# wushan270/mit-6.824-2015

Hardware: AMD Instinct MI355X
Metric: word-count input GB/s (whole node) and % of HBM roofline at 1/2/4/8 MI355X (higher is better)
Workload: dtype u8

## Files before the change

mit-6.824-2015_amd/csrc/wcg_agg.h:

```cpp
#pragma once
#include "wcg_common.h"
#include "wcg_lds_table.h"
#include "wcg_map.h"

namespace wcg {

constexpr int AGG_NT = 1024;
constexpr u32 AGG_BATCH = AGG_NT * 4;
constexpr int AGG_W = 2;
constexpr int AGG_NB = 3350;
constexpr u32 AGG_SLACK_UNITS = AGG_BATCH + 8;
constexpr u32 AGG_MAX_SRC = 256;
constexpr u32 AGG_Q = 128;
constexpr u32 AGG_OVF_CAP = 4096;
constexpr int AGG_SPILL = 0, AGG_EMIT = 1;
#ifndef WCG_AGG_PROBES
#define WCG_AGG_PROBES 2
#endif
constexpr int AGG_PROBES = WCG_AGG_PROBES;
#ifndef WCG_AGG_SPEC_K1
#define WCG_AGG_SPEC_K1 0
#endif
constexpr bool AGG_SPEC_K1 = WCG_AGG_SPEC_K1;
#ifndef WCG_AGG_SPEC_MED
// ... 3 lines not shown
#define WCG_AGG_KINDS 1
#endif
#ifndef WCG_AGG_ABLATE
#define WCG_AGG_ABLATE 0
#endif

struct AggArgs {
    const u64* pool;
    const u32* region_len;
    u64 region_cap;
    u32 P;
    u32 nsrc;
    u32 slices;
    u32 pm;
    u32 slices_m;
    u32 nbi;
    u32 ls_nreg;
    u32 rstride, rmod;
    u32 P1;
    int mode;
    GEntry* gtab;
    u64 gmask;
    DevState* st;
    const u64* map_stats;
    u64* spill;
    u64 spill_cap;
    u32* spill_len;
    Rec* emit;
    u64 emit_cap;
    Rec* ovf;
    u32 ovf_cap;
    u64* clk;
    uint16_t* flist;
};

#ifndef WCG_AGG2_LDSHASH
#define WCG_AGG2_LDSHASH 0
#endif
__device__ __forceinline__ u32 agg_hash(u64 k0, u64 k1) {
    if (WCG_AGG2_LDSHASH) return lds_hash(k0, k1) * 0x9E3779B1u;
    return (u32)(key_hash(k0, k1) >> 32);
}

__device__ __forceinline__ void agg_decode(const u64 (&u)[6], u64 (&k0)[4], u64 (&k1)[4], u64 (&c)[4], bool (&v)[4],
                                           u32 (&nu)[4]) {
#pragma unroll
    for (int k = 0; k < 4; k++) {
        const u32 T = (u32)(u[k] >> 56);
        const bool head = T >= 0x41;
        v[k] = T != 0 && (head || (T & 0x1F) < 8);
        const u64 last = head ? u[k + 1] : u[k];
        k0[k] = head ? u[k] : (u[k] & ~U_CNT);
        k1[k] = head ? (u[k + 1] & ~U_CNT) : 0;
        const bool hc = (last & U_CNT) != 0;
        c[k] = hc ? (head ? u[k + 2] : u[k + 1]) : 1;
        nu[k] = (head ? 2u : 1u) + (hc ? 1u : 0u);
    }
}

__device__ __forceinline__ void agg_decode_short(const u64 (&u)[6], u64 (&k0)[4], u64 (&k1)[4], u64 (&c)[4], bool (&v)[4],
                                                 u32 (&nu)[4]) {
#pragma unroll
    for (int k = 0; k < 4; k++) {
        v[k] = (u[k] >> 56) != 0;
        const bool hc = (u[k] & U_CNT) != 0;
        k0[k] = u[k] & ~U_CNT;
// ... 10 lines not shown
        const bool hc = (u[k + 1] & U_CNT) != 0;
        k0[k] = u[k];
        k1[k] = u[k + 1] & ~U_CNT;
        c[k] = hc ? u[k + 2] : 1;
        nu[k] = hc ? 3u : 2u;
    }
}

#define WCG_AGG_SET_OPS(S)                                                                      \
    __device__ __forceinline__ void agg_load_##S(const v4u* q, v4u& x0, v4u& x1, v4u& x2) {     \
        asm volatile("global_load_dwordx4 %0, %3, off ; wcg-load " #S "0\n\t"                   \
                     "global_load_dwordx4 %1, %3, off offset:16 ; wcg-load " #S "1\n\t"         \
                     "global_load_dwordx4 %2, %3, off offset:32 ; wcg-load " #S "2"              \
                     : "=&v"(x0), "=&v"(x1), "=&v"(x2) : "v"(q) : "memory");                    \
    }                                                                                           \
    template <int N>                                                                            \
    __device__ __forceinline__ void agg_wait_##S(v4u& x0, v4u& x1, v4u& x2) {                   \
        asm volatile("s_waitcnt vmcnt(%3) ; wcg-wait " #S " %0 %1 %2"                            \
                     : "+v"(x0), "+v"(x1), "+v"(x2) : "n"(N) : "memory");                       \
    }
WCG_AGG_SET_OPS(A)
WCG_AGG_SET_OPS(B)
WCG_AGG_SET_OPS(C)
#undef WCG_AGG_SET_OPS
#ifndef WCG_AGG_SETS1
#define WCG_AGG_SETS1 2
#endif
#ifndef WCG_AGG_SETS2
#define WCG_AGG_SETS2 2
#endif

template <int MODE, int KIND>
__device__ __forceinline__ u64 agg_one(const AggArgs& a, u32 bi, u64 (*tk0)[AGG_W], u64 (*tk1)[AGG_W], u64 (*tcnt)[AGG_W], u32* rlen_s,
                       u32* bstart, u32& spos, u64 (*wsum)[4]) {
    const int tid = threadIdx.x;
    LdsTable<AGG_NB, u64, AGG_W> tab{tk0, tk1, tcnt};
    constexpr bool emit = MODE == AGG_EMIT;
    u32 p, s, sl;
    if (bi < a.pm * a.slices) { p = bi % a.pm; s = bi / a.pm; sl = a.slices; }
    else { const u32 b2 = bi - a.pm * a.slices, nm = a.P - a.pm; p = a.pm + b2 % nm; s = b2 / nm; sl = a.slices_m; }
#ifdef WCG_AGG_MREV
    if (p >= a.pm && a.pm < a.P) p = a.P - 1 - (p - a.pm);
#endif
    u32 k0_, k1_, wbase, wstep;
    if (!emit) {
        k0_ = (u32)(((u64)a.nsrc * s) / sl); k1_ = (u32)(((u64)a.nsrc * (s + 1)) / sl);
        wbase = 0; wstep = 1;
    } else {
        k0_ = 0; k1_ = a.nsrc;
        wbase = p / AGG_Q; wstep = a.P1;
    }
    const u32 nk = k1_ - k0_;
    auto region = [&](u32 k) -> u64 { return (u64)(wbase + k * wstep) * a.rstride + p % a.rmod; };
    constexpr u32 WB = 256;
    for (u32 k = tid; k < nk; k += AGG_NT) rlen_s[k] = a.region_len[region(k0_ + k)];
    __syncthreads();
    if (tid == 0) {
        u32 t = 0;
        for (u32 k = 0; k < nk; k++) { bstart[k] = t; t += (rlen_s[k] + WB - 1) / WB; }
        bstart[nk] = t;
        spos = 0;
    }
    __syncthreads();
    const u32 nbat = bstart[nk];
    if (nbat == 0) {
        if (!emit && tid == 0 && a.spill_len) a.spill_len[bi] = 0;
        return 0;
    }
    tab.init(tid, AGG_NT);
    __syncthreads();
    u64 my_global = 0;
    u64* const sp = emit ? nullptr : a.spill + (u64)bi * a.spill_cap;
    auto overflow = [&](u64 k0, u64 k1, u64 c, u32 nu) {
        if (emit) {
            const u32 pos = atomicAdd(&spos, 1u);
            if (pos < a.ovf_cap) { a.ovf[(u64)blockIdx.x * a.ovf_cap + pos] = inline_rec(k0, k1, c); return; }
        } else {
            const u32 pos = atomicAdd(&spos, nu);
            if (pos + nu <= a.spill_cap) {
                u64 e[3];
                const u64 f = c > 1 ? U_CNT : 0;
                if (key_short(k0)) { e[0] = k0 | f; e[1] = c; }
                else { e[0] = k0; e[1] = k1 | f; e[2] = c; }
                for (u32 j = 0; j < nu; j++) sp[pos + j] = e[j];
                return;
            }
            for (u64 j = pos; j < a.spill_cap; j++) sp[j] = 0;
        }
        my_global++;
        ginsert(a.gtab, a.gmask, k0, k1, gslot(key_hash(k0, k1)), c, a.st);
    };
    const u32 wave = (u32)__builtin_amdgcn_readfirstlane(tid >> 6), lane = tid & 63;
    constexpr u32 WSTRIDE = AGG_NT / 64;
    const bool per_wave = !emit;
    auto advance = [&](u32& k, u32& b, u32 step) {
        if (per_wave) {
            b += step / WSTRIDE;
            while (k < nk && b >= bstart[k + 1] - bstart[k]) { k += WSTRIDE; b = 0; }
            return;
        }
        b += step;
        while (k < nk) {
            const u32 nbk = bstart[k + 1] - bstart[k];
            if (b < nbk) break;
            b -= nbk;
            k++;
        }
    };
    auto batch_ptr = [&](u32 k, u32 b) -> const v4u* {
        const bool live = k < nk;
        const u64 i = (live ? (u64)b * WB : 0) + 4 * lane;
        return reinterpret_cast<const v4u*>(a.pool + region(k0_ + (live ? k : 0)) * a.region_cap + i);
    };
    auto unit = [](const v4u& x, int h) -> u64 { return h ? ((u64)x.w << 32 | x.z) : ((u64)x.y << 32 | x.x); };
    auto process = [&](u32 k, u32 b, const v4u& x0, const v4u& x1, const v4u& x2) {
        u64 u[6] = {unit(x0, 0), unit(x0, 1), unit(x1, 0), unit(x1, 1), unit(x2, 0), unit(x2, 1)};
        const u32 i0 = b * WB + 4 * lane, len = rlen_s[k];
#pragma unroll
        for (int j = 0; j < 6; j++) u[j] = i0 + j < len ? u[j] : 0;
        if (WCG_AGG_ABLATE == 1) { asm volatile("" ::"v"(u[0] ^ u[1] ^ u[2] ^ u[3] ^ u[4] ^ u[5])); return; }
        u64 k0[4], k1[4], c[4];
        bool v[4];
        u32 nu[4];
        if (KIND == 1) agg_decode_short(u, k0, k1, c, v, nu);
        else if (KIND == 2) agg_decode_medium(u, k0, k1, c, v, nu);
        else agg_decode(u, k0, k1, c, v, nu);
        if (WCG_AGG_ABLATE == 4) {
#pragma unroll
            for (int j = 0; j < 4; j++) v[j] = v[j] && key_short(k0[j]);
        }
        if (WCG_AGG_ABLATE == 2) {
            u32 x = 0;
#pragma unroll
            for (int j = 0; j < 4; j++) x ^= v[j] ? lds_hash(k0[j], k1[j]) + (u32)c[j] : 0u;
            asm volatile("" ::"v"(x));
            return;
        }
        static_assert(4 % AGG_PROBES == 0, "probe groups split a lane's 4 units");
        constexpr bool SPEC = KIND == 2 ? WCG_AGG_SPEC_MED : AGG_SPEC_K1;
#pragma unroll
        for (int j = 0; j < 4; j += AGG_PROBES) {
            typename decltype(tab)::Probe pr[AGG_PROBES];
#pragma unroll
            for (int q = 0; q < AGG_PROBES; q++) {
                const u32 h = emit ? agg_hash(k0[j + q], k1[j + q]) : lds_hash(k0[j + q], k1[j + q]);
                if (!v[j + q]) continue;
                if (SPEC) tab.start_k1(h, KIND == 2 || !key_short(k0[j + q]), pr[q]);
                else tab.start(h, pr[q]);
            }
#pragma unroll
            for (int q = 0; q < AGG_PROBES; q++) {
                if (!v[j + q]) continue;
                const bool ok = SPEC ? tab.template finish_k1<KIND>(k0[j + q], k1[j + q], pr[q], c[j + q])
                                     : tab.template finish<KIND>(k0[j + q], k1[j + q], pr[q], c[j + q]);
                if (!ok) overflow(k0[j + q], k1[j + q], c[j + q], nu[j + q]);
            }
        }
    };
    constexpr int NSETS = emit ? WCG_AGG_SETS2 : WCG_AGG_SETS1;
    static_assert(NSETS == 2 || NSETS == 3, "k_agg's batch walk names two or three register sets");
    u32 kA = 0, bA = 0, kB, bB, kC = 0, bC = 0;
    if (per_wave) { kA = wave; bA = (u32)-1; advance(kA, bA, WSTRIDE); }
    else advance(kA, bA, wave);
    kB = kA; bB = bA;
    advance(kB, bB, WSTRIDE);
    v4u a0, a1, a2, b0, b1, b2, c0, c1, c2;
    agg_load_A(batch_ptr(kA, bA), a0, a1, a2);
    agg_load_B(batch_ptr(kB, bB), b0, b1, b2);
    if (NSETS == 3) {
        kC = kB; bC = bB;
        advance(kC, bC, WSTRIDE);
        agg_load_C(batch_ptr(kC, bC), c0, c1, c2);
        while (kA < nk) {
            agg_wait_A<6>(a0, a1, a2);
            process(kA, bA, a0, a1, a2);
            kA = kC; bA = bC;
            advance(kA, bA, WSTRIDE);
            agg_load_A(batch_ptr(kA, bA), a0, a1, a2);
            if (kB >= nk) break;
            agg_wait_B<6>(b0, b1, b2);
            process(kB, bB, b0, b1, b2);
            kB = kA; bB = bA;
            advance(kB, bB, WSTRIDE);
            agg_load_B(batch_ptr(kB, bB), b0, b1, b2);
            if (kC >= nk) break;
            agg_wait_C<6>(c0, c1, c2);
            process(kC, bC, c0, c1, c2);
            kC = kB; bC = bB;
            advance(kC, bC, WSTRIDE);
            agg_load_C(batch_ptr(kC, bC), c0, c1, c2);
        }
        agg_wait_C<0>(c0, c1, c2);
    } else {
        while (kA < nk) {
            agg_wait_A<3>(a0, a1, a2);
            process(kA, bA, a0, a1, a2);
            kA = kB; bA = bB;
            advance(kA, bA, WSTRIDE);
            agg_load_A(batch_ptr(kA, bA), a0, a1, a2);
            if (kB >= nk) break;
            agg_wait_B<3>(b0, b1, b2);
            process(kB, bB, b0, b1, b2);
            kB = kA; bB = bA;
            advance(kB, bB, WSTRIDE);
            agg_load_B(batch_ptr(kB, bB), b0, b1, b2);
        }
    }
    agg_wait_A<0>(a0, a1, a2);
    agg_wait_B<0>(b0, b1, b2);
    __syncthreads();
    if (!emit && a.flist && !a.spill_cap && WCG_AGG_ABLATE != 3) {
        constexpr u32 NE = AGG_NB * AGG_W;
        uint16_t* const L = a.flist + (u64)bi * NE;
        u32 mine = 0;
        for (int i = tid; i < (int)NE; i += AGG_NT) mine += (&tcnt[0][0])[i] ? 1u : 0u;
        u32 incl = mine;
        for (int d = 1; d < 64; d <<= 1) { const u32 y = __shfl_up(incl, d, 64); if (lane >= (u32)d) incl += y; }
        if (lane == 63) wsum[wave][0] = incl;
        __syncthreads();
        u32 pos = 0, all = 0;
        for (u32 w = 0; w < AGG_NT / 64; w++) { if (w < wave) pos += (u32)wsum[w][0]; all += (u32)wsum[w][0]; }
        pos += incl - mine;
        for (int i = tid; i < (int)NE; i += AGG_NT)
            if ((&tcnt[0][0])[i]) L[pos++] = (uint16_t)i;
        asm volatile("s_waitcnt vmcnt(0)" ::: "memory");
        __syncthreads();
        for (u32 j = tid; j < all; j += AGG_NT) {
            const u32 i = __hip_atomic_load(&L[j], __ATOMIC_RELAXED, __HIP_MEMORY_SCOPE_AGENT);
            const u64 c = (&tcnt[0][0])[i], k0 = (&tk0[0][0])[i], k1 = (&tk1[0][0])[i];
            my_global++;
            ginsert(a.gtab, a.gmask, k0, k1, gslot(key_hash(k0, k1)), c, a.st);
        }
        __syncthreads();
    } else if (!emit) {
        for (int i = tid; i < AGG_NB * AGG_W; i += AGG_NT) {
            const u64 c = (&tcnt[0][0])[i];
            if (!c || WCG_AGG_ABLATE == 3) continue;
            const u64 k0 = (&tk0[0][0])[i], k1 = (&tk1[0][0])[i];
            if (a.spill_cap) { overflow(k0, k1, c, (u32)entry_units(k0, (u32)(c > 1 ? 2 : 1))); continue; }
            my_global++;
            ginsert(a.gtab, a.gmask, k0, k1, gslot(key_hash(k0, k1)), c, a.st);
        }
        __syncthreads();
        if (tid == 0 && a.spill_len) a.spill_len[bi] = spos < a.spill_cap ? spos : (u32)a.spill_cap;
    } else {
        u32 mine = 0;
// ... 23 lines not shown
        for (int i = tid; i < AGG_NB * AGG_W; i += AGG_NT) {
            const u64 c = (&tcnt[0][0])[i];
            if (!c) continue;
            const u64 k0 = (&tk0[0][0])[i], k1 = (&tk1[0][0])[i];
            if (pos < a.emit_cap) a.emit[pos] = inline_rec(k0, k1, c);
            else { my_global++; ginsert(a.gtab, a.gmask, k0, k1, gslot(key_hash(k0, k1)), c, a.st); }
            pos++;
        }
    }
    __syncthreads();
    return my_global;
}

struct AggTabs {
    u64 tk0[AGG_NB][AGG_W];
    u64 tk1[AGG_NB][AGG_W];
    u64 tcnt[AGG_NB][AGG_W];
};
union AggLds {
    AggTabs t;
    LsLds ls;
};
static_assert(LS_NT == AGG_NT, "long_small runs as a k_agg workgroup");
template <int MODE>
__global__ __launch_bounds__(AGG_NT) void k_agg(AggArgs a, MapArgs ma) {
    __shared__ __align__(16) AggLds lds;
    u64 (*const tk0)[AGG_W] = lds.t.tk0;
    u64 (*const tk1)[AGG_W] = lds.t.tk1;
    u64 (*const tcnt)[AGG_W] = lds.t.tcnt;
    __shared__ u32 rlen_s[AGG_MAX_SRC];
    __shared__ u32 bstart[AGG_MAX_SRC + 1];
    __shared__ u32 spos;
    __shared__ u64 wsum[AGG_NT / 64][4];
    const int tid = threadIdx.x;
    const u32 nb = a.nbi;
    if (MODE == AGG_SPILL && a.ls_nreg && blockIdx.x == nb) {
        long_small(ma, a.ls_nreg, lds.ls);
        return;
    }
    const u64 t0 = a.clk ? wall_clock64() : 0;
    if (MODE == AGG_SPILL && blockIdx.x == 0 && tid == 0) { a.st->nrec = 0; a.st->nlong = 0; }
    u64 my_global = 0;
    for (u32 bi = blockIdx.x; bi < nb; bi += gridDim.x)
        if (MODE == AGG_SPILL && WCG_AGG_KINDS && a.pm < a.P)
            my_global += bi < a.pm * a.slices ? agg_one<MODE, 1>(a, bi, tk0, tk1, tcnt, rlen_s, bstart, spos, wsum)
                                              : agg_one<MODE, 2>(a, bi, tk0, tk1, tcnt, rlen_s, bstart, spos, wsum);
        else
            my_global += agg_one<MODE, 0>(a, bi, tk0, tk1, tcnt, rlen_s, bstart, spos, wsum);
    for (int d = 32; d >= 1; d >>= 1) my_global += __shfl_xor(my_global, d, 64);
    u64 ms = 0;
    if (blockIdx.x == 0 && MODE != AGG_EMIT)
        for (u32 w = tid >> 2; w < a.nsrc; w += AGG_NT / 4) ms += a.map_stats[(u64)w * 4 + (tid & 3)];
    for (int d = 32; d >= 4; d >>= 1) ms += __shfl_xor(ms, d, 64);
    if ((tid & 63) < 4) wsum[tid >> 6][tid & 3] = ms + ((tid & 63) == 2 ? my_global : 0);
    __syncthreads();
    if (tid < 4) {
        u64 t = 0;
        for (int w = 0; w < AGG_NT / 64; w++) t += wsum[w][tid];
        u64* dst[4] = {&a.st->tokens, &a.st->lds_hits, &a.st->global_ops, &a.st->long_tokens};
        if (t) atomicAdd(dst[tid], t);
    }
    if (a.clk && tid == 0) { a.clk[2 * blockIdx.x] = t0; a.clk[2 * blockIdx.x + 1] = wall_clock64(); }
}

#ifndef WCG_RP_QB
#define WCG_RP_QB 48
#endif
#ifndef WCG_RP_PREFETCH
#define WCG_RP_PREFETCH 0
#endif
constexpr u32 RP_QB = WCG_RP_QB;
struct RpArgs {
    const u64* pool; const u32* region_len; u64 region_cap;
    u32 P, nsrc, slices;
    const u64* map_stats;
    u64* pool2; u64 cap2; u32* region_len2;
    GEntry* gtab; u64 gmask; DevState* st;
};
#ifndef WCG_RP_MINB
#define WCG_RP_MINB 1
#endif
__global__ __launch_bounds__(AGG_NT, WCG_RP_MINB) void k_rp(RpArgs a) {
    __shared__ u64 sbuf[AGG_Q][RP_QB];
    __shared__ u32 scnt[AGG_Q], sfill[AGG_Q], gpos[AGG_Q], gbase[AGG_Q];
    __shared__ u32 sdirect[AGG_Q];
    __shared__ u64 wsum[AGG_NT / 64][4];
    const u32 b = blockIdx.x, tid = threadIdx.x;
    const u32 p = b % a.P, sl = b / a.P;
    const u32 k0_ = (u32)(((u64)a.nsrc * sl) / a.slices), k1_ = (u32)(((u64)a.nsrc * (sl + 1)) / a.slices);
    u64* const pool2 = a.pool2;
    const u64 cap2 = a.cap2;
    GEntry* const gtab = a.gtab;
    const u64 gmask = a.gmask;
    DevState* const st = a.st;
    if (b == 0) {
// ... 121 lines not shown
```

mit-6.824-2015_amd/csrc/wcg_api.hip:

```cpp
#include <hip/hip_ext.h>
#include <hip/hip_runtime.h>
#include <rccl/rccl.h>

#include <fcntl.h>
#include <sys/stat.h>
#include <unistd.h>

#include <algorithm>
#include <array>
#include <chrono>
#include <cstdio>
#include <cstdlib>
#include <cstring>
#include <memory>
#include <string>
#include <thread>
#include <tuple>
#include <vector>

#include "../../include/wcg.h"
#include "wcg_common.h"
#include "wcg_map.h"
#include "wcg_agg.h"
#include "wcg_reduce.h"
// ... 126 lines not shown
    u64* wg_stats = nullptr; u64 wg_stats_cap = 0;
    u64* llog = nullptr; u64 llog_cap = 0;
    u32* llog_len = nullptr; u64 llog_len_cap = 0;
    u64 chunk = 64ull << 20;
    uint8_t* hb[INGEST_SLOTS] = {};
    uint8_t* db[INGEST_SLOTS] = {};
    uint8_t* dbig = nullptr; u64 dbig_cap = 0;
    hipEvent_t ev_copied[INGEST_SLOTS] = {}, ev_mapped[INGEST_SLOTS] = {};
    std::vector<hipEvent_t> ing_ev;
    double ing[3] = {};
    u64 ing_chunks = 0;
    hipStream_t copy_stream = nullptr;
    std::unique_ptr<TaskPool> readers;
    u64 ingest_bytes = 0;
    bool timing = false;
    bool timing_all = false;
    std::vector<hipEvent_t> ev_pool;
    size_t ev_used = 0;
    std::vector<std::pair<hipEvent_t, hipEvent_t>> map_ev, agg_ev;
    hipEvent_t phase_ev[6] = {};
    u64 map_launches_since_reset = 0;
    int timing_mode = 0;
    std::vector<std::array<hipEvent_t, 5>> phase_jobs;
    bool phase_rec = false;
    std::vector<std::tuple<int, hipEvent_t, hipEvent_t>> xev;
    double acc[10] = {};
    u64 map_launches = 0;
    uint8_t* fr_buf = nullptr;
    FrArgs fr{};
    u32 fr_epoch = 0;
    bool fused_last = false;
    bool pending = false;
    uint16_t* flist = nullptr; u64 flist_cap = 0;
    u64* h_st_dev = nullptr;
    u64* seed = nullptr;
    bool seed_ok = false;
    double seed_rate = -1.0;
    bool job_seeded = false, job_unseeded = false, job_built = false;
    bool last_seeded = false;
    u64 seed_builds = 0;
    u64* d_clk = nullptr;
    u64* d_fclk = nullptr;
    u64* d_stamps = nullptr;
    std::string err;
};

namespace {

#define HIPCHK(ctx, call)                                                                   \
    do {                                                                                    \
        hipError_t e_ = (call);                                                             \
        if (e_ != hipSuccess) {                                                             \
            (ctx)->err = std::string(#call) + ": " + hipGetErrorString(e_);                 \
            return WCG_EHIP;                                                                \
        }                                                                                   \
    } while (0)

#define RC(call)                                                                            \
    do {                                                                                    \
        int rc_ = (call);                                                                   \
        if (rc_) return rc_;                                                                \
    } while (0)

u64 next_pow2(u64 x) {
    u64 p = 1;
    while (p < x) p <<= 1;
// ... 855 lines not shown
    HIPCHK(c, hipMalloc(&c->recA, c->rec_cap * sizeof(Rec)));
    HIPCHK(c, hipMalloc(&c->recB, c->rec_cap * sizeof(Rec)));
    HIPCHK(c, hipHostMalloc(&c->h_cur, EX_MAX_RANKS * sizeof(u64), hipHostMallocDefault));
    HIPCHK(c, hipMalloc(&c->d_per_rank, 2 * EX_MAX_RANKS * sizeof(u64)));
    return wcg_reset(c);
}

int wcg_close(wcg_ctx* c) {
    if (!c) return WCG_EINVAL;
    (void)hipSetDevice(c->device);
    if (c->stream) (void)hipStreamSynchronize(c->stream);
    if (c->copy_stream) (void)hipStreamSynchronize(c->copy_stream);
    if (c->long_stream) (void)hipStreamSynchronize(c->long_stream);
    c->readers.reset();
    if (c->ev_fork) (void)hipEventDestroy(c->ev_fork);
    if (c->ev_join) (void)hipEventDestroy(c->ev_join);
    for (auto e : c->ev_pool) (void)hipEventDestroy(e);
    for (int i = 0; i < INGEST_SLOTS; i++) {
        if (c->ev_copied[i]) (void)hipEventDestroy(c->ev_copied[i]);
    for (auto e : c->ing_ev) (void)hipEventDestroy(e);
        if (c->ev_mapped[i]) (void)hipEventDestroy(c->ev_mapped[i]);
        if (c->hb[i]) (void)hipHostFree(c->hb[i]);
        if (c->db[i]) (void)hipFree(c->db[i]);
    }
    void* bufs[] = {c->gtab, c->ltab, c->arena, c->st, c->recA, c->recB, c->lens, c->d_out,
                    c->d_part, c->owner, c->d_per_rank, c->exp_buf, c->pool, c->region_len, c->wg_stats,
                    c->llog, c->llog_len, c->smp, c->bid, c->spx, c->irec, c->lent, c->lpcur, c->spill, c->spill_len, c->pool2, c->rlen2, c->remit, c->ovf, c->hist, c->spart, c->ikey, c->iidx, c->groups,
                    c->pid, c->d_partb, c->nlpos, c->d_rb, c->d_b0, c->d_jin, c->d_jout, c->jhist, c->dbig,
                    c->ij_in, c->ij_tiles, c->ij_keys, c->ij_units,
                    c->d_xrow, c->xrecv, c->grecv, c->glist, c->llist, c->fr_buf, c->flist,
                    c->top_cand, c->top_rec, c->d_top, c->q_keys, c->q_off, c->q_cnt, c->rs_part, c->d_range,
                    c->bc_key[0], c->bc_key[1], c->bc_idx[0], c->bc_idx[1], c->bc_hist, c->bc_thist, c->bc_rec, c->d_bc,
                    c->bc_q, c->bc_r,
                    c->seed, c->d_clk, c->d_fclk, c->d_stamps};
    for (auto e : c->bc_ev) (void)hipEventDestroy(e);
    if (c->comm) (void)ncclCommDestroy(c->comm);
    for (void* b : bufs) if (b) (void)hipFree(b);
    if (c->h_x) (void)hipHostFree(c->h_x);
    if (c->h_st) (void)hipHostFree(c->h_st);
    if (c->h_cur) (void)hipHostFree(c->h_cur);
    if (c->h_rb) (void)hipHostFree(c->h_rb);
    if (c->copy_stream) (void)hipStreamDestroy(c->copy_stream);
    if (c->own_stream) (void)hipStreamDestroy(c->own_stream);
    if (c->long_stream) (void)hipStreamDestroy(c->long_stream);
    delete c;
    return WCG_OK;
}

int wcg_set_stream(wcg_ctx* c, void* stream) {
    if (!c) return WCG_EINVAL;
    hipStream_t next = stream ? (hipStream_t)stream : c->own_stream;
    if (next != c->stream) {
        int rc = set_dev(c);
        if (rc) return rc;
        hipEvent_t e;
        HIPCHK(c, hipEventCreateWithFlags(&e, hipEventDisableTiming));
        hipError_t r1 = hipEventRecord(e, c->stream);
        hipError_t r2 = r1 == hipSuccess ? hipStreamWaitEvent(next, e, 0) : r1;
        (void)hipEventDestroy(e);
        HIPCHK(c, r2);
        c->stream = next;
    }
    return WCG_OK;
}

int wcg_enable_timing(wcg_ctx* c, int on) {
    if (!c) return WCG_EINVAL;
// ... 63 lines not shown
        }
    }
    const u64* llist = nullptr;
    u64 l16 = c->lslots * sizeof(GEntry) / 16;
    if (c->llist && c->ltab_zero) {
        if (!touched) l16 = 0;
        else {
            RC(read_st());
            if (c->h_st->lnew <= LLIST_CAP) { llist = c->llist; l16 = 2 * c->h_st->lnew; }
        }
    }
    c->map_launches_since_reset = 0;
    if (!clear_g) g16 = 0;
    static_assert(sizeof(GEntry) == 32, "k_clear's listed entries are two 16-byte words");
    static const char* cg_env = getenv("WCG_CLEAR_GRID");
    const u64 cgrid = cg_env ? std::max<u64>(1, (u64)atoi(cg_env)) : grid_for(g16 + l16, 256, c->ncu * 4);
    k_clear<<<(unsigned)cgrid, 256, 0, c->stream>>>(
        reinterpret_cast<uint4*>(c->gtab), g16, reinterpret_cast<uint4*>(c->ltab), l16, c->st, glist, llist);
    HIPCHK(c, hipGetLastError());
    c->gtab_zero = true;
    c->ltab_zero = true;
    c->counts_clean = true;
    c->compacted = c->reduced = c->merged = false;
    c->exp_ready = false;
    c->part_R = 0; c->top_n = 0; c->range_ok = false; c->bc_ok = false; c->bcw_ok = false;
    c->nrec = 0;
    c->out_len = 0;
    c->two_pass_used = false;
    c->imported = false;
    return WCG_OK;
}

int agg_clock_report(wcg_ctx* c, const AggArgs& g, u32 nb1, u64 grid) {
    std::vector<u64> clk(2 * nb1);
    std::vector<u32> rl(grid * g.P);
    HIPCHK(c, hipMemcpyAsync(clk.data(), g.clk, clk.size() * sizeof(u64), hipMemcpyDeviceToHost, c->stream));
    HIPCHK(c, hipMemcpyAsync(rl.data(), g.region_len, rl.size() * sizeof(u32), hipMemcpyDeviceToHost, c->stream));
    HIPCHK(c, hipStreamSynchronize(c->stream));
    u64 t0 = ~0ull, t1 = 0;
    for (u32 b = 0; b < nb1; b++) { t0 = std::min(t0, clk[2 * b]); t1 = std::max(t1, clk[2 * b + 1]); }
    double sd = 0, su = 0, md = 0, mu = 0;
    double kd[2] = {0, 0}, km[2] = {0, 0}, ku[2] = {0, 0};
    u32 kn[2] = {0, 0};
    u32 bmax = 0;
    std::vector<u64> units(nb1, 0);
    for (u32 bi = 0; bi < nb1; bi++) {
        u32 p, s, sl;
        if (bi < g.pm * g.slices) { p = bi % g.pm; s = bi / g.pm; sl = g.slices; }
        else { const u32 b2 = bi - g.pm * g.slices, nm = g.P - g.pm; p = g.pm + b2 % nm; s = b2 / nm; sl = g.slices_m; }
        const u32 k0 = (u32)((grid * s) / sl), k1 = (u32)((grid * (s + 1)) / sl);
        for (u32 k = k0; k < k1; k++) units[bi] += rl[(u64)k * g.P + p];
        const double d = (double)(clk[2 * bi + 1] - clk[2 * bi]);
        sd += d; su += (double)units[bi];
        if (d > md) { md = d; bmax = bi; }
        mu = std::max(mu, (double)units[bi]);
        const int kind = bi >= g.pm * g.slices;
        kd[kind] += d; km[kind] = std::max(km[kind], d); ku[kind] += (double)units[bi]; kn[kind]++;
    }
    static const char* dump = getenv("WCG_AGG_CLOCK_DUMP");
    if (dump) {
        if (FILE* f = fopen(dump, "a")) {
            for (u32 bi = 0; bi < nb1; bi++)
                fprintf(f, "%u %u %llu %.2f %.2f\n", bi, (u32)(bi >= g.pm * g.slices), (unsigned long long)units[bi],
                        (clk[2 * bi] - t0) / 100.0, (clk[2 * bi + 1] - clk[2 * bi]) / 100.0);
            fprintf(f, "--\n");
            fclose(f);
        }
    }
    {
        std::vector<u32> ord(nb1);
        for (u32 i = 0; i < nb1; i++) ord[i] = i;
        std::sort(ord.begin(), ord.end(), [&](u32 x, u32 y) { return clk[2 * x + 1] - clk[2 * x] > clk[2 * y + 1] - clk[2 * y]; });
        for (u32 r = 0; r < std::min<u32>(5, nb1); r++) {
            const u32 bi = ord[r];
            fprintf(stderr, "wcg k_agg clock: slow #%u bi %u (%s) dur %.1f us units %llu\n", r, bi,
                    bi >= g.pm * g.slices ? "medium" : "short", (clk[2 * bi + 1] - clk[2 * bi]) / 100.0,
                    (unsigned long long)units[bi]);
        }
    }
    for (int kind = 0; kind < 2; kind++)
        if (kn[kind])
            fprintf(stderr, "wcg k_agg clock: %s workgroups %u, dur mean %.1f max %.1f us, units mean %.0f\n",
                    kind ? "medium" : "short", kn[kind], kd[kind] / kn[kind] / 100.0, km[kind] / 100.0, ku[kind] / kn[kind]);
    fprintf(stderr, "wcg k_agg clock: span %.1f us, wg dur mean %.1f max %.1f us (bi %u: %llu units, start +%.1f us), "
            "units mean %.0f max %.0f\n", (t1 - t0) / 100.0, sd / nb1 / 100.0, md / 100.0, bmax,
            (unsigned long long)units[bmax], (clk[2 * bmax] - t0) / 100.0, su / nb1, mu);
    return WCG_OK;
}

}

extern "C" {

int wcg_reset(wcg_ctx* c) {
    if (!c) return WCG_EINVAL;
    c->pending = false;
    c->job_seeded = c->job_unseeded = c->job_built = false;
    int rc = set_dev(c);
    if (rc) return rc;
    if (c->timing_mode >= 2 && c->ev_used >= EV_FOLD) {
        HIPCHK(c, hipStreamSynchronize(c->stream));
        sum_events(c, c->acc);
        c->map_ev.clear(); c->agg_ev.clear(); c->phase_jobs.clear(); c->xev.clear();
        c->ev_used = 0;
    }
    RC(reset_tables(c));
    if (c->timing_mode < 2) {
        c->map_ev.clear();
        c->agg_ev.clear();
        c->xev.clear();
        c->ev_used = 0;
// ... 171 lines not shown
    g.P = P; g.nsrc = (u32)grid;
    const u32 min_sl = (u32)((grid + AGG_MAX_SRC - 1) / AGG_MAX_SRC);
    if (split) {
        g.pm = MISS_SHORT_BUCKETS;
        const u32 nm = P - g.pm;
        static const char* ms_env = getenv("WCG_AGG_MSLICES");
        g.slices_m = std::max<u32>(min_sl, std::max<u32>(1, std::min<u32>((u32)grid,
                                   ms_env ? (u32)atoi(ms_env) : (u32)c->ncu / 4 / nm)));
        g.slices = std::max<u32>(min_sl, std::max<u32>(1, std::min<u32>((u32)grid,
                                 (u32)(c->ncu > g.slices_m * nm ? (c->ncu - g.slices_m * nm) / g.pm : 1))));
    } else {
        g.pm = P;
        g.slices_m = 1;
        g.slices = std::max<u32>(1, std::min<u32>((u32)grid, (u32)(c->ncu + P - 1) / P));
        g.slices = std::max<u32>(g.slices, min_sl);
    }
    g.nbi = g.pm * g.slices + (P - g.pm) * g.slices_m;
    g.ls_nreg = small ? (u32)grid : 0u;
    g.rstride = P; g.rmod = P; g.P1 = P; g.mode = AGG_SPILL;
    g.gtab = c->gtab; g.gmask = c->gslots - 1; g.st = c->st;
    g.map_stats = c->wg_stats;
    const u32 nb1 = g.nbi;
    g.spill_cap = 0;
    g.spill = nullptr; g.spill_len = nullptr;
    g.emit = c->remit; g.emit_cap = rec_cap_emit;
    g.ovf = nullptr; g.ovf_cap = 0;
    g.clk = nullptr;
    g.flist = nullptr;
    static const char* fl_env = getenv("WCG_AGG_FLIST");
    if (!two_pass && !(fl_env && atoi(fl_env) == 0)) {
        RC(ensure(c, &c->flist, &c->flist_cap, (u64)nb1 * AGG_NB * AGG_W));
        g.flist = c->flist;
    }
    static const bool agg_clock = getenv("WCG_AGG_CLOCK") != nullptr;
    u64*& d_clk = c->d_clk;
    if (agg_clock && !two_pass) {
        if (!d_clk) HIPCHK(c, hipMalloc(&d_clk, 2 * 65536 * sizeof(u64)));
        g.clk = nb1 <= 65536 ? d_clk : nullptr;
    }
    if (!two_pass) {
        k_agg<AGG_SPILL><<<nb1 + (small ? 1 : 0), AGG_NT, 0, c->stream>>>(g, a);
        HIPCHK(c, hipGetLastError());
        c->counts_clean = true;
        if (g.clk) RC(agg_clock_report(c, g, nb1, grid));
    } else {
    c->two_pass_used = true;
    static const char* rps_env = getenv("WCG_RP_SLICES");
    const u32 sl = std::max<u32>(1, std::min<u32>((u32)grid, rps_env ? (u32)atoi(rps_env) : 2 * g.slices));
    const u32 nrp = P * sl;
    const u64 slice_cap = (u64)cdiv(grid, sl) * a.region_cap;
    u64 cap2 = ((slice_cap * 3 / 2) / AGG_Q + 1024) & ~1ull;
    u64 cap2_env;
    if (cap_env("WCG_RP_CAP2", &cap2_env)) cap2 = std::max<u64>(2, std::min<u64>(cap2_env, 1ull << 31)) & ~1ull;
    RC(ensure(c, &c->pool2, &c->pool2_cap, (u64)nrp * AGG_Q * cap2 + AGG_SLACK_UNITS));
    RC(ensure(c, &c->rlen2, &c->rlen2_cap, (u64)nrp * AGG_Q));
    RpArgs rp;
    rp.pool = c->pool; rp.region_len = c->region_len; rp.region_cap = a.region_cap;
    rp.P = P; rp.nsrc = (u32)grid; rp.slices = sl; rp.map_stats = c->wg_stats;
    rp.pool2 = c->pool2; rp.cap2 = cap2; rp.region_len2 = c->rlen2;
    rp.gtab = c->gtab; rp.gmask = c->gslots - 1; rp.st = c->st;
    k_rp<<<nrp, AGG_NT, 0, c->stream>>>(rp);
    AggArgs g2 = g;
    g2.pool = c->pool2; g2.region_len = c->rlen2; g2.region_cap = cap2;
    g2.P = P * AGG_Q; g2.nsrc = sl; g2.slices = 1;
    g2.pm = g2.P; g2.slices_m = 1; g2.nbi = g2.P;
    g2.rstride = AGG_Q; g2.rmod = AGG_Q; g2.P1 = P; g2.mode = AGG_EMIT;
    const u32 grid2 = std::min<u32>(P * AGG_Q, (u32)c->ncu * 2);
    g2.ovf_cap = AGG_OVF_CAP;
    RC(ensure(c, &c->ovf, &c->ovf_cap, (u64)grid2 * AGG_OVF_CAP));
    g2.ovf = c->ovf;
    g2.ls_nreg = 0;
    k_agg<AGG_EMIT><<<grid2, AGG_NT, 0, c->stream>>>(g2, a);
    HIPCHK(c, hipGetLastError());
    }
// ... 1425 lines not shown
```

Baseline: 1194.

## Add dynamic work-stealing walk to k_agg spill pass with cross-partition helping

Replaces the static slice assignment in the aggregation spill kernel with a per-partition atomic cursor. Workgroups claim chunks of quarter-region items, and workgroups that finish early help the partition with the most remaining work. The long_small path is handed to the first workgroup that wins a ticket instead of getting its own extra block. This targets load imbalance from skewed partitions, at the cost of global atomics, more LDS-table merges when helpers spill the same partition, and a last-block reset of the cursors.

```diff
diff --git a/mit-6.824-2015_amd/csrc/wcg_agg.h b/mit-6.824-2015_amd/csrc/wcg_agg.h
--- a/mit-6.824-2015_amd/csrc/wcg_agg.h
+++ b/mit-6.824-2015_amd/csrc/wcg_agg.h
@@ -59,6 +59,27 @@
     u32 ovf_cap;
     u64* clk;
     uint16_t* flist;
+    u32* cur;
+    u32 help_min;
+};
+
+#ifndef WCG_AGG_PARTS_LOG2
+#define WCG_AGG_PARTS_LOG2 2
+#endif
+constexpr u32 AGG_PARTS_LOG2 = WCG_AGG_PARTS_LOG2, AGG_PARTS = 1u << AGG_PARTS_LOG2;
+static_assert(AGG_PARTS <= 16, "a bucket's items fit 16 bits of lq and 24 of best");
+constexpr u32 AGG_CLAIM = 16;
+constexpr u32 AGG_CLK_WGS = 65536, AGG_CLK_DYN = 2 * AGG_CLK_WGS;
+constexpr u32 AGG_HELP_MIN = 16;
+constexpr u32 AGG_CUR_DONE = MAX_MISS_BUCKETS, AGG_CUR_TICKET = MAX_MISS_BUCKETS + 1, AGG_CUR_WORDS = MAX_MISS_BUCKETS + 2;
+struct AggDyn {
+    u32 lq;
+    u32 lock;
+    u32 dry;
+    u32 nclaim;
+    u32 best;
+    u32 tk;
+    u32 dg[4];
 };
 
 #ifndef WCG_AGG2_LDSHASH
@@ -135,8 +156,9 @@
 
 template <int MODE, int KIND>
 __device__ __forceinline__ u64 agg_one(const AggArgs& a, u32 bi, u64 (*tk0)[AGG_W], u64 (*tk1)[AGG_W], u64 (*tcnt)[AGG_W], u32* rlen_s,
-                       u32* bstart, u32& spos, u64 (*wsum)[4]) {
+                       u32* bstart, u32& spos, u64 (*wsum)[4], AggDyn& dy) {
     const int tid = threadIdx.x;
+    const bool dyn = MODE == AGG_SPILL && a.cur != nullptr;
     LdsTable<AGG_NB, u64, AGG_W> tab{tk0, tk1, tcnt};
     constexpr bool emit = MODE == AGG_EMIT;
     u32 p, s, sl;
@@ -146,7 +168,10 @@
     if (p >= a.pm && a.pm < a.P) p = a.P - 1 - (p - a.pm);
 #endif
     u32 k0_, k1_, wbase, wstep;
-    if (!emit) {
+    if (dyn) {
+        k0_ = 0; k1_ = a.nsrc;
+        wbase = 0; wstep = 1;
+    } else if (!emit) {
         k0_ = (u32)(((u64)a.nsrc * s) / sl); k1_ = (u32)(((u64)a.nsrc * (s + 1)) / sl);
         wbase = 0; wstep = 1;
     } else {
@@ -154,8 +179,24 @@
         wbase = p / AGG_Q; wstep = a.P1;
     }
     const u32 nk = k1_ - k0_;
+    const u32 sh = dyn ? AGG_PARTS_LOG2 : 0u, nki = nk << sh;
     auto region = [&](u32 k) -> u64 { return (u64)(wbase + k * wstep) * a.rstride + p % a.rmod; };
     constexpr u32 WB = 256;
+    if (dyn) {
+        u32 any = 0;
+        for (u32 k = tid; k < nk; k += AGG_NT) { const u32 l = a.region_len[region(k)]; rlen_s[k] = l; any |= l; }
+        any = __syncthreads_or((int)any);
+        if (tid == 0) {
+            const u32 base = atomicAdd(&a.cur[p], any ? AGG_CLAIM : nki);
+            const bool got = any && base < nki;
+            dy.lq = got ? base | (base + AGG_CLAIM < nki ? base + AGG_CLAIM : nki) << 16 : 0u;
+            dy.dry = got ? 0u : 1u;
+            dy.lock = 0; dy.nclaim = 0;
+            spos = 0;
+        }
+        __syncthreads();
+        if (dy.dry) return 0;
+    } else {
     for (u32 k = tid; k < nk; k += AGG_NT) rlen_s[k] = a.region_len[region(k0_ + k)];
     __syncthreads();
     if (tid == 0) {
@@ -165,7 +206,8 @@
         spos = 0;
     }
     __syncthreads();
-    const u32 nbat = bstart[nk];
+    }
+    const u32 nbat = dyn ? 1u : bstart[nk];
     if (nbat == 0) {
         if (!emit && tid == 0 && a.spill_len) a.spill_len[bi] = 0;
         return 0;
@@ -196,10 +238,49 @@
     const u32 wave = (u32)__builtin_amdgcn_readfirstlane(tid >> 6), lane = tid & 63;
     constexpr u32 WSTRIDE = AGG_NT / 64;
     const bool per_wave = !emit;
+    u32 nreg = 0;
+    auto ibeg = [&](u32 k) -> u32 { return (((rlen_s[k >> sh] + WB - 1) / WB) * (k & ((1u << sh) - 1))) >> sh; };
+    auto iend = [&](u32 k) -> u32 { return (((rlen_s[k >> sh] + WB - 1) / WB) * ((k & ((1u << sh) - 1)) + 1)) >> sh; };
+    auto take = [&]() -> u32 {
+        u32 r = nki;
+        if (lane == 0) {
+            u32 q = atomicAdd(&dy.lq, 1u);
+            if ((q & 0xFFFF) < (q >> 16)) r = q & 0xFFFF;
+            else if (!*(volatile u32*)&dy.dry) {
+                if (atomicExch(&dy.lock, 1u) == 0) {
+                    q = atomicAdd(&dy.lq, 1u);
+                    if ((q & 0xFFFF) < (q >> 16)) r = q & 0xFFFF;
+                    else {
+                        const u32 base = atomicAdd(&a.cur[p], AGG_CLAIM);
+                        if (base < nki) {
+                            r = base;
+                            atomicExch(&dy.lq, (base + 1) | (base + AGG_CLAIM < nki ? base + AGG_CLAIM : nki) << 16);
+                        } else *(volatile u32*)&dy.dry = 1;
+                    }
+                    atomicExch(&dy.lock, 0u);
+                } else {
+                    const u32 base = atomicAdd(&a.cur[p], 1u);
+                    if (base < nki) r = base;
+                    else *(volatile u32*)&dy.dry = 1;
+                }
+            }
+        }
+        return (u32)__builtin_amdgcn_readfirstlane(r);
+    };
+    auto take_region = [&]() -> u32 {
+        u32 k;
+        do k = take(); while (k < nki && ibeg(k) == iend(k));
+        if (k < nki) nreg++;
+        return k;
+    };
     auto advance = [&](u32& k, u32& b, u32 step) {
         if (per_wave) {
-            b += step / WSTRIDE;
-            while (k < nk && b >= bstart[k + 1] - bstart[k]) { k += WSTRIDE; b = 0; }
+            if (k >= nki) return;
+            b++;
+            if (b < iend(k)) return;
+            if (dyn) k = take_region();
+            else do k += WSTRIDE; while (k < nk && rlen_s[k] == 0);
+            b = k < nki ? ibeg(k) : 0u;
             return;
         }
         b += step;
@@ -211,14 +292,14 @@
         }
     };
     auto batch_ptr = [&](u32 k, u32 b) -> const v4u* {
-        const bool live = k < nk;
+        const bool live = k < nki;
         const u64 i = (live ? (u64)b * WB : 0) + 4 * lane;
-        return reinterpret_cast<const v4u*>(a.pool + region(k0_ + (live ? k : 0)) * a.region_cap + i);
+        return reinterpret_cast<const v4u*>(a.pool + region(k0_ + (live ? k >> sh : 0)) * a.region_cap + i);
     };
     auto unit = [](const v4u& x, int h) -> u64 { return h ? ((u64)x.w << 32 | x.z) : ((u64)x.y << 32 | x.x); };
     auto process = [&](u32 k, u32 b, const v4u& x0, const v4u& x1, const v4u& x2) {
         u64 u[6] = {unit(x0, 0), unit(x0, 1), unit(x1, 0), unit(x1, 1), unit(x2, 0), unit(x2, 1)};
-        const u32 i0 = b * WB + 4 * lane, len = rlen_s[k];
+        const u32 i0 = b * WB + 4 * lane, len = rlen_s[k >> sh];
 #pragma unroll
         for (int j = 0; j < 6; j++) u[j] = i0 + j < len ? u[j] : 0;
         if (WCG_AGG_ABLATE == 1) { asm volatile("" ::"v"(u[0] ^ u[1] ^ u[2] ^ u[3] ^ u[4] ^ u[5])); return; }
@@ -263,7 +344,8 @@
     constexpr int NSETS = emit ? WCG_AGG_SETS2 : WCG_AGG_SETS1;
     static_assert(NSETS == 2 || NSETS == 3, "k_agg's batch walk names two or three register sets");
     u32 kA = 0, bA = 0, kB, bB, kC = 0, bC = 0;
-    if (per_wave) { kA = wave; bA = (u32)-1; advance(kA, bA, WSTRIDE); }
+    if (dyn) { kA = take_region(); bA = kA < nki ? ibeg(kA) : 0u; }
+    else if (per_wave) { kA = wave; bA = (u32)-1; advance(kA, bA, WSTRIDE); }
     else advance(kA, bA, wave);
     kB = kA; bB = bA;
     advance(kB, bB, WSTRIDE);
@@ -274,19 +356,19 @@
         kC = kB; bC = bB;
         advance(kC, bC, WSTRIDE);
         agg_load_C(batch_ptr(kC, bC), c0, c1, c2);
-        while (kA < nk) {
+        while (kA < nki) {
             agg_wait_A<6>(a0, a1, a2);
             process(kA, bA, a0, a1, a2);
             kA = kC; bA = bC;
             advance(kA, bA, WSTRIDE);
             agg_load_A(batch_ptr(kA, bA), a0, a1, a2);
-            if (kB >= nk) break;
+            if (kB >= nki) break;
             agg_wait_B<6>(b0, b1, b2);
             process(kB, bB, b0, b1, b2);
             kB = kA; bB = bA;
             advance(kB, bB, WSTRIDE);
             agg_load_B(batch_ptr(kB, bB), b0, b1, b2);
-            if (kC >= nk) break;
+            if (kC >= nki) break;
             agg_wait_C<6>(c0, c1, c2);
             process(kC, bC, c0, c1, c2);
             kC = kB; bC = bB;
@@ -295,13 +377,13 @@
         }
         agg_wait_C<0>(c0, c1, c2);
     } else {
-        while (kA < nk) {
+        while (kA < nki) {
             agg_wait_A<3>(a0, a1, a2);
             process(kA, bA, a0, a1, a2);
             kA = kB; bA = bB;
             advance(kA, bA, WSTRIDE);
             agg_load_A(batch_ptr(kA, bA), a0, a1, a2);
-            if (kB >= nk) break;
+            if (kB >= nki) break;
             agg_wait_B<3>(b0, b1, b2);
             process(kB, bB, b0, b1, b2);
             kB = kA; bB = bA;
@@ -311,10 +393,11 @@
     }
     agg_wait_A<0>(a0, a1, a2);
     agg_wait_B<0>(b0, b1, b2);
+    if (dyn && lane == 0 && nreg) atomicAdd(&dy.nclaim, nreg);
     __syncthreads();
     if (!emit && a.flist && !a.spill_cap && WCG_AGG_ABLATE != 3) {
         constexpr u32 NE = AGG_NB * AGG_W;
-        uint16_t* const L = a.flist + (u64)bi * NE;
+        uint16_t* const L = a.flist + (u64)blockIdx.x * NE;
         u32 mine = 0;
         for (int i = tid; i < (int)NE; i += AGG_NT) mine += (&tcnt[0][0])[i] ? 1u : 0u;
         u32 incl = mine;
@@ -404,21 +487,68 @@
     __shared__ u32 bstart[AGG_MAX_SRC + 1];
     __shared__ u32 spos;
     __shared__ u64 wsum[AGG_NT / 64][4];
+    __shared__ AggDyn dy;
     const int tid = threadIdx.x;
     const u32 nb = a.nbi;
-    if (MODE == AGG_SPILL && a.ls_nreg && blockIdx.x == nb) {
-        long_small(ma, a.ls_nreg, lds.ls);
-        return;
-    }
+    const bool dyn = MODE == AGG_SPILL && a.cur != nullptr;
+    bool ls_now = MODE == AGG_SPILL && !dyn && a.ls_nreg && blockIdx.x == nb;
     const u64 t0 = a.clk ? wall_clock64() : 0;
     if (MODE == AGG_SPILL && blockIdx.x == 0 && tid == 0) { a.st->nrec = 0; a.st->nlong = 0; }
     u64 my_global = 0;
-    for (u32 bi = blockIdx.x; bi < nb; bi += gridDim.x)
+    bool first = true;
+    if (dyn && tid == 0) { dy.dg[0] = dy.dg[1] = dy.dg[2] = dy.dg[3] = 0; }
+    for (u32 bi = blockIdx.x; ls_now || bi < nb;) {
+        if (MODE == AGG_SPILL && ls_now) {
+            long_small(ma, a.ls_nreg, lds.ls);
+            if (!dyn) return;
+            ls_now = false;
+            if (tid == 0) dy.dg[3] = 1;
+        } else {
         if (MODE == AGG_SPILL && WCG_AGG_KINDS && a.pm < a.P)
-            my_global += bi < a.pm * a.slices ? agg_one<MODE, 1>(a, bi, tk0, tk1, tcnt, rlen_s, bstart, spos, wsum)
-                                              : agg_one<MODE, 2>(a, bi, tk0, tk1, tcnt, rlen_s, bstart, spos, wsum);
+            my_global += bi < a.pm * a.slices ? agg_one<MODE, 1>(a, bi, tk0, tk1, tcnt, rlen_s, bstart, spos, wsum, dy)
+                                              : agg_one<MODE, 2>(a, bi, tk0, tk1, tcnt, rlen_s, bstart, spos, wsum, dy);
         else
-            my_global += agg_one<MODE, 0>(a, bi, tk0, tk1, tcnt, rlen_s, bstart, spos, wsum);
+            my_global += agg_one<MODE, 0>(a, bi, tk0, tk1, tcnt, rlen_s, bstart, spos, wsum, dy);
+        if (!dyn) { bi += gridDim.x; continue; }
+        if (tid == 0) {
+            const u32 got = dy.nclaim;
+            if (first) dy.dg[0] = got;
+            else { dy.dg[1] += got; dy.dg[2] += got ? 1u : 0u; }
+        }
+        const bool ls_open = first && a.ls_nreg != 0;
+        first = false;
+        if (ls_open) {
+            if (tid == 0)
+                dy.tk = __hip_atomic_load(&a.cur[AGG_CUR_TICKET], __ATOMIC_RELAXED, __HIP_MEMORY_SCOPE_AGENT) ? 1u
+                                                                                                             : atomicAdd(&a.cur[AGG_CUR_TICKET], 1u);
+            __syncthreads();
+            if (dy.tk == 0) { ls_now = true; continue; }
+        }
+        }
+        if (tid == 0) dy.best = 0;
+        __syncthreads();
+        if ((u32)tid < a.P) {
+            const u32 c = __hip_atomic_load(&a.cur[tid], __ATOMIC_RELAXED, __HIP_MEMORY_SCOPE_AGENT);
+            if (c < a.nsrc << AGG_PARTS_LOG2) atomicMax(&dy.best, ((a.nsrc << AGG_PARTS_LOG2) - c) << 8 | (u32)tid);
+        }
+        __syncthreads();
+        const u32 best = dy.best;
+        if ((best >> 8) < a.help_min) break;
+        const u32 hp = best & 255;
+        bi = hp < a.pm ? hp : a.pm * a.slices + (hp - a.pm);
+    }
+    if (dyn) {
+        __syncthreads();
+        if (tid == 0) {
+            __threadfence();
+            dy.tk = atomicAdd(&a.cur[AGG_CUR_DONE], 1u);
+        }
+        __syncthreads();
+        if (dy.tk == gridDim.x - 1) {
+            __threadfence();
+            for (u32 i = tid; i < AGG_CUR_WORDS; i += AGG_NT) a.cur[i] = 0;
+        }
+    }
     for (int d = 32; d >= 1; d >>= 1) my_global += __shfl_xor(my_global, d, 64);
     u64 ms = 0;
     if (blockIdx.x == 0 && MODE != AGG_EMIT)
@@ -432,7 +562,13 @@
         u64* dst[4] = {&a.st->tokens, &a.st->lds_hits, &a.st->global_ops, &a.st->long_tokens};
         if (t) atomicAdd(dst[tid], t);
     }
-    if (a.clk && tid == 0) { a.clk[2 * blockIdx.x] = t0; a.clk[2 * blockIdx.x + 1] = wall_clock64(); }
+    if (a.clk && tid == 0) {
+        a.clk[2 * blockIdx.x] = t0; a.clk[2 * blockIdx.x + 1] = wall_clock64();
+        if (dyn) {
+            a.clk[AGG_CLK_DYN + 2 * blockIdx.x] = dy.dg[0] | (u64)dy.dg[1] << 32;
+            a.clk[AGG_CLK_DYN + 2 * blockIdx.x + 1] = dy.dg[2] | (u64)dy.dg[3] << 32;
+        }
+    }
 }
 
 #ifndef WCG_RP_QB
diff --git a/mit-6.824-2015_amd/csrc/wcg_api.hip b/mit-6.824-2015_amd/csrc/wcg_api.hip
--- a/mit-6.824-2015_amd/csrc/wcg_api.hip
+++ b/mit-6.824-2015_amd/csrc/wcg_api.hip
@@ -182,6 +182,7 @@
     bool fused_last = false;
     bool pending = false;
     uint16_t* flist = nullptr; u64 flist_cap = 0;
+    u32* agg_cur = nullptr;
     u64* h_st_dev = nullptr;
     u64* seed = nullptr;
     bool seed_ok = false;
@@ -1103,7 +1104,7 @@
                     c->top_cand, c->top_rec, c->d_top, c->q_keys, c->q_off, c->q_cnt, c->rs_part, c->d_range,
                     c->bc_key[0], c->bc_key[1], c->bc_idx[0], c->bc_idx[1], c->bc_hist, c->bc_thist, c->bc_rec, c->d_bc,
                     c->bc_q, c->bc_r,
-                    c->seed, c->d_clk, c->d_fclk, c->d_stamps};
+                    c->seed, c->agg_cur, c->d_clk, c->d_fclk, c->d_stamps};
     for (auto e : c->bc_ev) (void)hipEventDestroy(e);
     if (c->comm) (void)ncclCommDestroy(c->comm);
     for (void* b : bufs) if (b) (void)hipFree(b);
@@ -1233,9 +1234,10 @@
 }
 
 int agg_clock_report(wcg_ctx* c, const AggArgs& g, u32 nb1, u64 grid) {
-    std::vector<u64> clk(2 * nb1);
+    std::vector<u64> clk(2 * nb1), dg(2 * nb1, 0);
     std::vector<u32> rl(grid * g.P);
     HIPCHK(c, hipMemcpyAsync(clk.data(), g.clk, clk.size() * sizeof(u64), hipMemcpyDeviceToHost, c->stream));
+    if (g.cur) HIPCHK(c, hipMemcpyAsync(dg.data(), g.clk + AGG_CLK_DYN, dg.size() * sizeof(u64), hipMemcpyDeviceToHost, c->stream));
     HIPCHK(c, hipMemcpyAsync(rl.data(), g.region_len, rl.size() * sizeof(u32), hipMemcpyDeviceToHost, c->stream));
     HIPCHK(c, hipStreamSynchronize(c->stream));
     u64 t0 = ~0ull, t1 = 0;
@@ -1262,8 +1264,9 @@
     if (dump) {
         if (FILE* f = fopen(dump, "a")) {
             for (u32 bi = 0; bi < nb1; bi++)
-                fprintf(f, "%u %u %llu %.2f %.2f\n", bi, (u32)(bi >= g.pm * g.slices), (unsigned long long)units[bi],
-                        (clk[2 * bi] - t0) / 100.0, (clk[2 * bi + 1] - clk[2 * bi]) / 100.0);
+                fprintf(f, "%u %u %llu %.2f %.2f %u %u %u %u\n", bi, (u32)(bi >= g.pm * g.slices), (unsigned long long)units[bi],
+                        (clk[2 * bi] - t0) / 100.0, (clk[2 * bi + 1] - clk[2 * bi]) / 100.0, (u32)dg[2 * bi],
+                        (u32)(dg[2 * bi] >> 32), (u32)dg[2 * bi + 1], (u32)(dg[2 * bi + 1] >> 32));
             fprintf(f, "--\n");
             fclose(f);
         }
@@ -1274,10 +1277,26 @@
         std::sort(ord.begin(), ord.end(), [&](u32 x, u32 y) { return clk[2 * x + 1] - clk[2 * x] > clk[2 * y + 1] - clk[2 * y]; });
         for (u32 r = 0; r < std::min<u32>(5, nb1); r++) {
             const u32 bi = ord[r];
-            fprintf(stderr, "wcg k_agg clock: slow #%u bi %u (%s) dur %.1f us units %llu\n", r, bi,
+            fprintf(stderr, "wcg k_agg clock: slow #%u bi %u (%s) dur %.1f us units %llu", r, bi,
                     bi >= g.pm * g.slices ? "medium" : "short", (clk[2 * bi + 1] - clk[2 * bi]) / 100.0,
                     (unsigned long long)units[bi]);
-        }
+            if (g.cur)
+                fprintf(stderr, " items home %u help %u joins %u%s", (u32)dg[2 * bi], (u32)(dg[2 * bi] >> 32),
+                        (u32)dg[2 * bi + 1], dg[2 * bi + 1] >> 32 ? " long_small" : "");
+            fprintf(stderr, "\n");
+        }
+    }
+    if (g.cur) {
+        u64 home = 0, help = 0, joins = 0, helpers = 0;
+        long ls = -1;
+        for (u32 bi = 0; bi < nb1; bi++) {
+            home += (u32)dg[2 * bi]; help += dg[2 * bi] >> 32; joins += (u32)dg[2 * bi + 1];
+            helpers += (u32)dg[2 * bi + 1] ? 1 : 0;
+            if (dg[2 * bi + 1] >> 32) ls = bi;
+        }
+        fprintf(stderr, "wcg k_agg clock: dynamic walk, help_min %u items (1/%u regions): claimed at home %llu, helping %llu in %llu joins "
+                "by %llu workgroups, long_small run by workgroup %ld\n", g.help_min, AGG_PARTS, (unsigned long long)home,
+                (unsigned long long)help, (unsigned long long)joins, (unsigned long long)helpers, ls);
     }
     for (int kind = 0; kind < 2; kind++)
         if (kn[kind])
@@ -1515,14 +1534,26 @@
         RC(ensure(c, &c->flist, &c->flist_cap, (u64)nb1 * AGG_NB * AGG_W));
         g.flist = c->flist;
     }
+    g.cur = nullptr;
+    g.help_min = AGG_HELP_MIN << AGG_PARTS_LOG2;
+    const char* dyn_env = getenv("WCG_AGG_DYN");
+    if (!two_pass && grid <= AGG_MAX_SRC && nb1 >= P && !(dyn_env && atoi(dyn_env) == 0)) {
+        if (!c->agg_cur) {
+            HIPCHK(c, hipMalloc(&c->agg_cur, AGG_CUR_WORDS * sizeof(u32)));
+            HIPCHK(c, hipMemsetAsync(c->agg_cur, 0, AGG_CUR_WORDS * sizeof(u32), c->stream));
+        }
+        g.cur = c->agg_cur;
+        u64 hm;
+        if (cap_env("WCG_AGG_HELP_MIN", &hm)) g.help_min = (u32)std::min<u64>(std::max<u64>(1, hm), AGG_MAX_SRC + 1) << AGG_PARTS_LOG2;
+    }
     static const bool agg_clock = getenv("WCG_AGG_CLOCK") != nullptr;
     u64*& d_clk = c->d_clk;
     if (agg_clock && !two_pass) {
-        if (!d_clk) HIPCHK(c, hipMalloc(&d_clk, 2 * 65536 * sizeof(u64)));
-        g.clk = nb1 <= 65536 ? d_clk : nullptr;
+        if (!d_clk) HIPCHK(c, hipMalloc(&d_clk, 4 * AGG_CLK_WGS * sizeof(u64)));
+        g.clk = nb1 <= AGG_CLK_WGS ? d_clk : nullptr;
     }
     if (!two_pass) {
-        k_agg<AGG_SPILL><<<nb1 + (small ? 1 : 0), AGG_NT, 0, c->stream>>>(g, a);
+        k_agg<AGG_SPILL><<<nb1 + (small && !g.cur ? 1 : 0), AGG_NT, 0, c->stream>>>(g, a);
         HIPCHK(c, hipGetLastError());
         c->counts_clean = true;
         if (g.clk) RC(agg_clock_report(c, g, nb1, grid));
```

After: 1174. 0.983x the previous value.
